# borodark/exmc

Hardware: AMD Instinct MI355X
Metric: leapfrog_steps_per_s (higher is better)
Workload: dtype f64; 1 GPU; eight_schools d=10, 4096 chains/GPU (4096 total), 138450 draws/chain (2769 steps of 50 draws) after one shared 1000-iteration warmup, max_tree_depth 10, target_accept 0.8; draws_per_chain=138450, lanes_per_chain=16, warmup_lanes_per_chain=16, seed=42

## Files before the change

exmc_amd/csrc/exmc_models.hpp:

```cpp
#pragma once

#include "exmc_device.hpp"

namespace exmc {

__device__ __forceinline__ double clamp200(double z) { return fmax(-200.0, fmin(z, 200.0)); }

struct ModelDefaults {
  static constexpr bool kVregMath = false;
  static constexpr bool kCoop = false;
  static constexpr int kExtraLdsDoubles = 0;
  static constexpr int kStageDoubles = 0;
  template <class C>
  __host__ static bool stage_ok(const C&) { return true; }
  static constexpr int kStageRowOffset = 0;
  static constexpr int kLdsDataDoubles = 0;
  static constexpr bool kPipeWarmup = true;
  static constexpr bool kHasPipeWarmup = true;
  static constexpr bool kXRowLds = false;
  static constexpr bool kRowDense = false;
  static constexpr bool kLaneDense = false;
  static constexpr bool kDenseImage = false;
  static constexpr int kDenseLdsDoubles = 0;
  static constexpr int kNutsWavesPerSimd = 1;
  static constexpr bool kRngOrbit = false;
  static constexpr bool kMigrate = false;
  static constexpr double kPrioRateWith = 1.0, kPrioRateWithout = 1.0;
  static constexpr int kPipeNutsLevels = 0;
  static constexpr bool kNutsZigInLds = true;
  static constexpr bool kRegradProposal = false;
  static constexpr int kWgWaves = 0;
  static constexpr int kWgLdsLevels = 1;
  static constexpr int kWgImageDoubles = 0;
  template <class C>
  __host__ __device__ static bool wg_ok(const C&) { return false; }
  static constexpr bool kLeafPairs = false;
  static constexpr bool kLeafPairExp = false;
  static constexpr bool kLeanMomentum = false;
  static constexpr bool kPassExpPairs = false;
  static constexpr bool kOuterLogPair = false;
  static constexpr bool kTreePrefix = false;
};

extern __shared__ double exmc_dyn_lds[];
typedef double exmc_v2d __attribute__((ext_vector_type(2)));
typedef __attribute__((address_space(3))) exmc_v2d lds_v2d;
typedef __attribute__((address_space(3))) double lds_f64_m;
static __device__ const double exmc_logtab_dev[2 * EXMC_LOGTAB_ENTRIES] = {EXMC_LOGTAB_VALUES};
__device__ static __forceinline__ double exmc_log_tab_global(double x) {
  double m;
  int e;
  const int i = exmc_logtab_split(x, &m, &e);
  return exmc_logtab_finish(m, e, exmc_logtab_dev[2 * i], exmc_logtab_dev[2 * i + 1]);
}

struct EightSchoolsConsts {
  double y[8], sg[8], lsg[8];
  double c_mu;
  double c_hc;
  double c1;
};

template <int G>
struct EightSchools : ModelDefaults {
  static constexpr int D = 10;
  static constexpr int DPL = (D + G - 1) / G;
  static constexpr bool kVregMath = (DPL <= 2);
#ifndef EXMC_ES_PIPE_LEVELS
#define EXMC_ES_PIPE_LEVELS 2
#endif
  static constexpr int kPipeNutsLevels = (G == 16) ? EXMC_ES_PIPE_LEVELS : 0;
  static constexpr bool kLeafPairs = (G == 16);
  static constexpr bool kLeafPairExp = (G == 16);
  static constexpr bool kLeanMomentum = (G == 16);
  static constexpr bool kOuterLogPair = (G == 16);
  static constexpr bool kTreePrefix = (G == 16);
  using MM = Math<kVregMath>;
  using Consts = EightSchoolsConsts;
  struct Lane {
    double y[DPL], lsg[DPL];
    Recip sg[DPL];
    Recip five;
    double cc;
  };

  __device__ static __forceinline__ void load(const Consts& c, int l, Lane& ln) {
#pragma unroll
    for (int k = 0; k < DPL; k++) {
      const int i = l + k * G;
      const int j = (i >= 2 && i < D) ? (i - 2) : 0;
      ln.y[k] = c.y[j];
      ln.sg[k] = make_recip(c.sg[j]);
      ln.lsg[k] = c.lsg[j];
    }
    ln.five = make_recip_literal(5.0);
    ln.cc = (l == 0) ? c.c_mu : c.c1;
  }

  __device__ static __forceinline__ double logp_grad(const Consts& c, const Lane& ln, int l,
                                                     const double (&q)[DPL], double (&g)[DPL]) {
    return with_fast_div([&](auto& dv) -> double { return eval(c, ln, l, q, g, dv); });
  }

  template <class DV>
  __device__ static __forceinline__ double eval(const Consts& c, const Lane& ln, int l,
                                                const double (&q)[DPL], double (&g)[DPL], DV& dv) {
    if constexpr (kSeqSum<G, D>) return eval_row(c, ln, l, q, g, dv);
    else return eval_slots(c, ln, l, q, g, dv);
  }

  struct Mid {
    double den, zc, T, lik;
  };
  template <class DV>
  __device__ static __forceinline__ void eval_row_grad(const Consts& c, const Lane& ln, int l,
                                                       const double (&q)[DPL], double (&g)[DPL], DV& dv,
                                                       Mid& m) {
    static_assert(DPL == 1, "one dimension per lane");
    const double mu = group_bcast_c<G, 0>(q[0]);
    const double zraw = group_bcast_c<G, 1>(q[0]);
    const double zc = clamp200(zraw);
    const double tau = MM::exp_pm200(zc);
    const bool isth = (l >= 2) && (l < D);
    const bool l0 = (l == 0), l1 = (l == 1);
    const double th = q[0];
    const double theta = mu + tau * th;
    const double resid = ln.y[0] - theta;
    dv.watch_if(isth, resid);
    dv.watch_if(isth, ln.sg[0].b);
    const double z = dv(resid, ln.sg[0]);
    const double a = dv(z, ln.sg[0]);
    const double Lk = isth ? ((-0.5 * (z * z)) - ln.lsg[0]) : 0.0;
    const double Ak = isth ? a : 0.0;
    const double Bk = isth ? (a * th) : 0.0;
    double lik = 0.0, sa = 0.0, sb = 0.0;
    row_seqsum<D>(lik, sa, sb, Lk, Ak, Bk);
    const double x = l0 ? (mu - 0.0) : tau;
    dv.watch_if(l0, x);
    const double zh = dv(x, ln.five);
    const double zh2 = zh * zh;
    const double w = dv(zh, ln.five);
    const double den = 1.0 + zh2;
    const double dhc = -dv(2.0 * w, den);
    const bool in = (zraw > -200.0) && (zraw < 200.0);
    double g_tau = in ? ((dhc + sb) * tau + 1.0) : 0.0;
    __asm__("" : "+v"(g_tau));
    const double g_mu = (-w) + sa;
    const double g_th = (-th) + a * tau;
    const double u2 = l0 ? zh2 : (th * th);
    g[0] = l0 ? g_mu : (l1 ? g_tau : g_th);
    m.den = den;
    m.zc = zc;
    m.T = -0.5 * (u2 + ln.cc);
    m.lik = lik;
  }
  __device__ static __forceinline__ double eval_row_finish(const Consts& c, int l, const Mid& m, double lg) {
    double t_tau = (c.c_hc - lg) + m.zc;
    __asm__("" : "+v"(t_tau));
    const double T = (l == 1) ? t_tau : m.T;
// ... 1108 lines not shown
          for (int j = 0; j < kAhead - 1; j++) v[j] = *ad[j];
          __builtin_amdgcn_sched_barrier(0);
          exmc_wait_lgkm0();
#pragma unroll
          for (int j = 0; j < kAhead - 1; j++) sj = sj + v[j];
        }
        sj_own[k] = sj;
      }
    } else {
#pragma unroll
      for (int k = 0; k < DPL; k++) {
        double lik = 0.0, f = 0.0, z2s = 0.0, sj = 0.0;
        for (int i = ln.i0[k]; i < ln.i1[k]; i++) sj = sj + obs(alpha_own[k], c.fl[i], c.y[i], lik, f, z2s);
        sj_own[k] = sj;
        if (valid[k]) {
          s[0] = s[0] + lik;
          s[4] = s[4] + f;
          s[5] = s[5] + z2s;
        }
      }
    }
#pragma unroll
    for (int k = 0; k < DPL; k++) {
      const double ar = q[k];
      const double sj = sj_own[k];
      if (valid[k]) {
        s[1] = s[1] + sj;
        s[2] = s[2] + sj * ln.u[k];
        s[3] = s[3] + sj * ar;
      }
      T[k] = -0.5 * (ar * ar + ln.kc[kC1]);
      g[k] = (-ar) + sj * sa;
    }
    if constexpr (G == 64) rs64_allsum6(s);
    else group_allsum_n<G, 6>(s);
    const bool in_a = (zsa_raw > -200.0) && (zsa_raw < 200.0);
    const bool in_y = (zsy_raw > -200.0) && (zsy_raw < 200.0);
    if constexpr (kSpread) {
      constexpr int ks = J / G;
      const int j = l + ks * G;
      const bool is_mu = j == J, is_g = j == J + 1, is_a = j == J + 2, is_y = j == J + 3, is_b = j == J + 4;
      const double v = is_mu ? mu : (is_g ? gam : beta);
      Recip rc;
      rc.b = is_mu ? ln.ten.b : ln.five.b;
      rc.r = is_mu ? ln.ten.r : ln.five.r;
      const double cst = is_mu ? ln.kc[kMu10] : ln.kc[kN5];
      const double sx = is_mu ? s[1] : (is_g ? s[2] : s[4]);
      const double zn = dv(v - 0.0, rc);
      const double Tn = -0.5 * (zn * zn + cst);
      const double gn = (-dv(zn, rc)) + sx;
      const double zc = is_a ? za : zy, zc2 = is_a ? za2 : zy2;
      const double dc = -dv(dv(2.0 * zc, ln.c25), 1.0 + zc2);
      const double ga = in_a ? ((dc + s[3]) * sa + 1.0) : 0.0;
      const double gy = in_y ? ((dc * sy + s[5]) + 1.0) : 0.0;
      const bool is_n = is_mu || is_g || is_b;
      T[ks] = is_n ? Tn : (is_a ? t_sa : (is_y ? t_sy : T[ks]));
      g[ks] = is_n ? gn : (is_a ? ga : (is_y ? gy : g[ks]));
#pragma unroll
      for (int k = 0; k < DPL; k++)
        if (l + k * G >= D) g[k] = 0.0;
      return group_sum_slots<G, DPL>(T, valid, l, s[0]);
    }
    const double zmu = dv(mu - 0.0, ln.ten), zg = dv(gam - 0.0, ln.five), zb = dv(beta - 0.0, ln.five);
#pragma unroll
    for (int k = 0; k < DPL; k++) {
      const int j = l + k * G;
      if (j == J) { T[k] = -0.5 * (zmu * zmu + ln.kc[kMu10]); g[k] = (-dv(zmu, ln.ten)) + s[1]; }
      if (j == J + 1) { T[k] = -0.5 * (zg * zg + ln.kc[kN5]); g[k] = (-dv(zg, ln.five)) + s[2]; }
      if (j == J + 2) { T[k] = t_sa; g[k] = in_a ? ((dsa + s[3]) * sa + 1.0) : 0.0; }
      if (j == J + 3) { T[k] = t_sy; g[k] = in_y ? ((dsy * sy + s[5]) + 1.0) : 0.0; }
      if (j == J + 4) { T[k] = -0.5 * (zb * zb + ln.kc[kN5]); g[k] = (-dv(zb, ln.five)) + s[4]; }
      if (j >= D) g[k] = 0.0;
    }
    return group_sum_slots<G, DPL>(T, valid, l, s[0]);
  }
};

template <class M>
struct RowDenseModel : M {
  static constexpr bool kRowDense = true;
  static constexpr bool kPipeWarmup = false;
  static constexpr bool kOuterLogPair = false;
  static constexpr bool kTreePrefix = false;
  static_assert(M::DPL == 1 && M::D <= 12, "row layout: one dimension per lane, D <= 12");
};

template <class M, int G>
struct LaneDenseModel : M {
  static constexpr bool kLaneDense = true;
  static constexpr bool kPipeWarmup = false;
  static constexpr int kNutsWavesPerSimd = 1;
  static constexpr int kPipeNutsLevels = 0;
  static constexpr bool kDenseImage = M::D * M::D * 8 <= 16 * 1024;
  static constexpr int kDenseLdsDoubles = (64 / G) * 3 * M::D + (kDenseImage ? M::D * M::D + 64 : 0);
  static_assert(G >= 16 && M::DPL * G >= M::D && !M::kCoop, "a lane layout that holds the whole chain");
};

}

#ifdef EXMC_CUSTOM_HEADER
#define EXMC_GEN_HOST static inline
#define EXMC_GEN_FN static __host__ __device__ __forceinline__
static __host__ __device__ __noinline__ double exmc_gen_exp_call(double x) { return exmc_exp(x); }
static __host__ __device__ __noinline__ double exmc_gen_log_call(double x) { return exmc_log(x); }
static __host__ __device__ __noinline__ double exmc_gen_log1p_call(double x) { return exmc_log1p(x); }
static __host__ __device__ __noinline__ double exmc_gen_erf_call(double x) { return exmc_erf(x); }
#define EXMC_GEN_ERF exmc_gen_erf_call
#define EXMC_GENV_ERF exmc_gen_erf_call
#ifdef EXMC_GEN_INLINE_MATH
#define EXMC_GEN_EXP exmc_exp
#define EXMC_GEN_LOG exmc_log
#define EXMC_GEN_LOG1P exmc_log1p
#else
#define EXMC_GEN_EXP exmc_gen_exp_call
#define EXMC_GEN_LOG exmc_gen_log_call
#define EXMC_GEN_LOG1P exmc_gen_log1p_call
#endif
#ifdef EXMC_GENV_CALLED_MATH
#define EXMC_GENV_EXP exmc_gen_exp_call
#define EXMC_GENV_LOG exmc_gen_log_call
#define EXMC_GENV_LOG1P exmc_gen_log1p_call
#else
#define EXMC_GENV_EXP exmc_exp
#define EXMC_GENV_LOG exmc_log
#define EXMC_GENV_LOG1P exmc_log1p
#endif
#ifdef EXMC_GENL_CALLED_MATH
#define EXMC_GENL_EXP exmc_gen_exp_call
#define EXMC_GENL_LOG exmc_gen_log_call
#define EXMC_GENL_LOG1P exmc_gen_log1p_call
#else
#define EXMC_GENL_EXP exmc::Math<true>::exp
#define EXMC_GENL_LOG exmc::Math<true>::log
#define EXMC_GENL_LOG1P exmc_log1p
#endif
#define EXMC_GENL_ERF exmc_gen_erf_call
#define EXMC_GEN_CTX_DECL , int shoff
#define EXMC_GEN_SH(i) exmc::exmc_dyn_lds[shoff + (i)]
#define EXMC_GEN_XROW (EXMC_GEN_LANES == 64 && EXMC_GEN_WAVES_PER_SIMD == 2)
#define EXMC_GEN_ALLSUM(s) exmc::group_allsum_n<EXMC_GEN_LANES, EXMC_GEN_NS, EXMC_GEN_XROW>(s)
#define EXMC_GEN_ALLSUM_W(w) exmc::group_allsum_n<EXMC_GEN_LANES, EXMC_GEN_NW, EXMC_GEN_XROW>(w)
#define EXMC_GEN_BATCH_LOG(n, b) exmc::lane_batch<EXMC_GEN_LANES, n>(b, l, [](double a_) { return EXMC_GENL_LOG(a_); })
#define EXMC_GEN_BATCH_EXP(n, b) exmc::lane_batch<EXMC_GEN_LANES, n>(b, l, [](double a_) { return EXMC_GENL_EXP(a_); })
#define EXMC_GEN_BATCH_LOG1P(n, b) exmc::lane_batch<EXMC_GEN_LANES, n>(b, l, [](double a_) { return EXMC_GENL_LOG1P(a_); })
#define EXMC_GEN_BATCH_RCP(n, b) exmc::lane_batch<EXMC_GEN_LANES, n>(b, l, [](double a_) { return 1.0 / a_; })
#define EXMC_GEN_FENCE() exmc::wave_lds_fence()
#define EXMC_GEN_SCAN_FWD(N, v, m, zo, h, sg, wo)                              \
  do {                                                                        \
    exmc::wave_scan_fwd<N>(v);                                                \
    _Pragma("unroll") for (int k_ = 0; k_ < (N); k_++)                        \
      if (l + 64 * k_ <= (m)) EXMC_GEN_SH((wo) + l + 64 * k_) = (v)[k_];     \
    exmc::wave_lds_fence();                                                   \
  } while (0)
#define EXMC_GEN_SCAN_BWD(N, v, m, zo, sg, we, ww, ga, sz, a0)                 \
  do {                                                                        \
    exmc::wave_scan_bwd<N>(v);                                                \
    double p_[1] = {0.0};                                                     \
    _Pragma("unroll") for (int k_ = 0; k_ < (N); k_++) {                      \
      const int e_ = l + 64 * k_;                                             \
      const bool in_ = e_ >= 1 && e_ <= (m);                                  \
      const double z_ = EXMC_GEN_SH(EXMC_GEN_IT((zo) + e_));                  \
      if (in_) EXMC_GEN_SH((ga) + e_) = (sg) * (v)[k_];                       \
      p_[0] = in_ ? p_[0] + z_ * (v)[k_] : p_[0];                             \
    }                                                                         \
    exmc::group_allsum_n<64, 1, EXMC_GEN_XROW>(p_);                           \
    (sz) = p_[0];                                                             \
// ... 378 lines not shown
```

exmc_amd/csrc/exmc_nuts.hpp:

```cpp
#pragma once

#include <type_traits>

#include "exmc_models.hpp"

#ifndef EXMC_ABLATE
#define EXMC_ABLATE 0
#endif

#ifndef EXMC_PROFILE_SECTIONS
#define EXMC_PROFILE_SECTIONS 0
#endif

namespace exmc {

#ifdef EXMC_XCC_PROBE
__device__ double g_wave_probe[4096 * 5];
#endif

#if EXMC_PROFILE_SECTIONS
__device__ unsigned long long g_prof[16];
#define EXMC_PROF_DECL long long prof_[10] = {0, 0, 0, 0, 0, 0, 0, 0, 0, 0}; long long prof_t_ = clock64();
#define EXMC_PROF(i) { const long long n_ = clock64(); prof_[i] += n_ - prof_t_; prof_t_ = n_; }
#define EXMC_PROF_COUNT(i) { prof_[i] += 1; }
// ... 365 lines not shown
    const uint32_t h1 = (uint32_t)__builtin_amdgcn_ds_bpermute(src, (int)hi[1]);
    const bool up = p >= 64;
    return ((uint64_t)(up ? h1 : h0) << 32) | (uint64_t)(up ? l1 : l0);
  }
  __device__ __forceinline__ Rng state(int p) const {
    auto word = [&](int q) -> uint64_t {
      const int w = q >> 6, i = q & 63;
      const uint32_t l = (w == 0) ? __builtin_amdgcn_readlane((int)lo[0], i) : __builtin_amdgcn_readlane((int)lo[1], i);
      const uint32_t h = (w == 0) ? __builtin_amdgcn_readlane((int)hi[0], i) : __builtin_amdgcn_readlane((int)hi[1], i);
      return ((uint64_t)h << 32) | (uint64_t)l;
    };
    Rng r;
    r.b = word(p);
    r.a = (p == 0) ? a0 : word(p > 0 ? p - 1 : 0);
    return r;
  }
};

#ifndef EXMC_RNG_ORBIT_MARGIN
#define EXMC_RNG_ORBIT_MARGIN 16
#endif

template <class M, int G>
__device__ __forceinline__ void draw_momentum_orbit(const NutsLane<M, G>& L, Rng& rng, double (&z)[M::DPL]) {
  constexpr int D = M::D, DPL = M::DPL;
  constexpr int NORB = D + EXMC_RNG_ORBIT_MARGIN;
#pragma unroll
  for (int k = 0; k < DPL; k++) z[k] = 0.0;
  int pos = 0;
  for (;;) {
    RngOrbit<NORB> orb;
    orb.build(rng);
    const int org = pos;
    int shift = 0;
    bool rebuild = false;
    for (;;) {
      bool fail[DPL];
#pragma unroll
      for (int k = 0; k < DPL; k++) {
        const bool live = L.valid[k] && (L.rank[k] >= pos);
        const int pp = live ? (L.rank[k] - org + shift) : 0;
        double zz;
        const bool acc = normal_fast(rng_scramble(orb.at(pp)), L.zt, zz);
        fail[k] = live && !acc;
        z[k] = (live && acc) ? zz : z[k];
      }
      int j = D;
      if (L.perm == nullptr) {
#pragma unroll
        for (int k = DPL - 1; k >= 0; k--) {
          const unsigned long long m = __ballot(fail[k] ? 1 : 0);
          j = (m != 0) ? (k * G + __ffsll((long long)m) - 1) : j;
        }
      } else {
#pragma unroll
        for (int k = 0; k < DPL; k++) j = fail[k] ? min(j, L.rank[k]) : j;
        j = group_min_i32<G>(j);
      }
      j = __builtin_amdgcn_readfirstlane(j);
      if (j >= D) {
        rng = orb.state(D - org + shift);
        return;
      }
      Rng rj = orb.state(j - org + shift);
      int words = 0;
      const double zz = rng_normal_counted(rj, L.zt, L.nor_r, words);
#pragma unroll
      for (int k = 0; k < DPL; k++) z[k] = (L.rank[k] == j) ? zz : z[k];
      words = __builtin_amdgcn_readfirstlane(words);
      pos = j + 1;
      shift += words - 1;
      if (D - org + shift > NORB - 1) {
        rng = rj;
        rebuild = true;
        break;
      }
    }
    if (!rebuild) return;
    if (pos >= D) return;
  }
}

template <class M, int G>
__device__ __forceinline__ void draw_momentum_lean(const NutsLane<M, G>& L, Rng& rng,
                                                   double (&z)[M::DPL]) {
  constexpr int D = M::D, DPL = M::DPL;
  static_assert(G < 64, "the 64-lane layouts have the orbit form");
  const int base = (threadIdx.x & 63) & ~(G - 1);
#pragma unroll
  for (int k = 0; k < DPL; k++) z[k] = 0.0;
  int pos = 0;
  bool first = true;
  for (;;) {
    Rng r2 = rng;
    uint64_t sb[DPL];
#pragma unroll
    for (int k = 0; k < DPL; k++) sb[k] = 0;
    if (first) {
#pragma nounroll
      for (int i = 0; i < D; i++) {
#pragma unroll
        for (int k = 0; k < DPL; k++) sb[k] = (L.rank[k] == i) ? r2.b : sb[k];
        rng_advance(r2);
      }
    } else {
      const int i0 = wave_min_pos<G>(pos);
#pragma nounroll
      for (int i = i0; i < D; i++) {
        const bool act = i >= pos;
#pragma unroll
        for (int k = 0; k < DPL; k++) sb[k] = (act && (L.rank[k] == i)) ? r2.b : sb[k];
        Rng nx = r2;
        rng_advance(nx);
        r2.a = act ? nx.a : r2.a;
        r2.b = act ? nx.b : r2.b;
      }
    }
    first = false;
    bool fail[DPL];
#pragma unroll
    for (int k = 0; k < DPL; k++) {
      const bool live = L.valid[k] && (L.rank[k] >= pos);
      double zz;
      const bool acc = normal_fast(rng_scramble(sb[k]), L.zt, zz);
      fail[k] = live && !acc;
      z[k] = (live && acc) ? zz : z[k];
    }
    int j = D;
#pragma unroll
    for (int k = DPL - 1; k >= 0; k--) {
      const unsigned long long m = __ballot(fail[k] ? 1 : 0);
      const unsigned long long gm = (m >> base) & ((1ULL << G) - 1ULL);
      j = (gm != 0) ? (k * G + __ffsll((long long)gm) - 1) : j;
    }
    if (__any((j < D) ? 1 : 0) == 0) {
      rng = r2;
      break;
    }
    if (j < D) {
      const int jp = (j > pos) ? j - 1 : j;
      uint64_t bj = 0, bp = 0;
#pragma unroll
      for (int k = 0; k < DPL; k++) {
        bj = (k == j / G) ? sb[k] : bj;
        bp = (k == jp / G) ? sb[k] : bp;
      }
      Rng rj;
      rj.b = __shfl(bj, base | (j & (G - 1)), 64);
      const uint64_t hp = __shfl(bp, base | (jp & (G - 1)), 64);
      rj.a = (j > pos) ? hp : rng.a;
      const double zz = rng_normal(rj, L.zt, L.nor_r);
#pragma unroll
      for (int k = 0; k < DPL; k++) z[k] = (L.rank[k] == j) ? zz : z[k];
      rng = rj;
      pos = j + 1;
    } else {
      rng = r2;
      pos = D;
    }
  }
}

template <class M, int G>
__device__ __forceinline__ void draw_momentum_variates(const NutsLane<M, G>& L, Rng& rng,
                                                       double (&z)[M::DPL]) {
  constexpr int D = M::D, DPL = M::DPL;
  if constexpr (G == 64 && M::kRngOrbit && D + EXMC_RNG_ORBIT_MARGIN <= 128) {
    draw_momentum_orbit<M, G>(L, rng, z);
    return;
  }
  if constexpr (G < 64 && M::kLeanMomentum) {
    if (L.perm == nullptr) {
      draw_momentum_lean<M, G>(L, rng, z);
      return;
    }
  }
  const int base = (threadIdx.x & 63) & ~(G - 1);
#pragma unroll
  for (int k = 0; k < DPL; k++) z[k] = 0.0;
  int pos = 0;
  for (;;) {
    Rng r2 = rng;
    uint64_t sa[DPL], sb[DPL];
#pragma unroll
    for (int k = 0; k < DPL; k++) { sa[k] = 0; sb[k] = 0; }
    const int i0 = wave_min_pos<G>(pos);
#pragma nounroll
    for (int i = i0; i < D; i++) {
      const bool act = (G == 64) || (i >= pos);
#pragma unroll
      for (int k = 0; k < DPL; k++) {
        const bool mine = act && (L.rank[k] == i);
        sa[k] = mine ? r2.a : sa[k];
        sb[k] = mine ? r2.b : sb[k];
      }
      Rng nx = r2;
      rng_advance(nx);
      r2.a = act ? nx.a : r2.a;
      r2.b = act ? nx.b : r2.b;
    }
    bool fail[DPL];
#pragma unroll
    for (int k = 0; k < DPL; k++) {
      const bool live = L.valid[k] && (L.rank[k] >= pos);
      double zz;
      const bool acc = normal_fast(rng_scramble(sb[k]), L.zt, zz);
      fail[k] = live && !acc;
      z[k] = (live && acc) ? zz : z[k];
    }
    int j = D;
    if (L.perm == nullptr) {
#pragma unroll
      for (int k = DPL - 1; k >= 0; k--) {
        const unsigned long long m = __ballot(fail[k] ? 1 : 0);
        const unsigned long long gm = (G == 64) ? m : ((m >> base) & ((1ULL << (G & 63)) - 1ULL));
        j = (gm != 0) ? (k * G + __ffsll((long long)gm) - 1) : j;
      }
    } else {
#pragma unroll
      for (int k = 0; k < DPL; k++) j = fail[k] ? min(j, L.rank[k]) : j;
      j = group_min_i32<G>(j);
    }
    if (__any((j < D) ? 1 : 0) == 0) {
      rng = r2;
      break;
    }
    if (j < D) {
      const int dim = (L.perm == nullptr) ? j : L.perm[j];
      const int ks = dim / G;
      uint64_t aj = 0, bj = 0;
#pragma unroll
      for (int k = 0; k < DPL; k++) {
        aj = (k == ks) ? sa[k] : aj;
        bj = (k == ks) ? sb[k] : bj;
      }
      const int src = base | (dim & (G - 1));
      Rng rj;
      rj.a = __shfl(aj, src, 64);
      rj.b = __shfl(bj, src, 64);
      const double zz = rng_normal(rj, L.zt, L.nor_r);
#pragma unroll
      for (int k = 0; k < DPL; k++) z[k] = (L.rank[k] == j) ? zz : z[k];
// ... 332 lines not shown
#pragma unroll
    for (int k = 0; k < DPL; k++) {
      const double ph = p[k] + h * g[k];
      p[k] = ph;
      q[k] = q[k] + eps_dir * (im[k] * ph);
    }
    f.logp = M::logp_grad(mc, L.ln, L.l, q, g);
#pragma unroll
    for (int k = 0; k < DPL; k++) p[k] = p[k] + h * g[k];
    const double jlp = f.logp - kinetic_energy<G, DPL, M::D, M::kXRowLds>(p, im, L.valid);
    const bool fin = exmc_isfinite(jlp);
    const double dl = jlp - jlp0;
    f.div = fin ? (dl < -1000.0) : true;
    f.lsw = fin ? dl : -1001.0;
    f.acc = f.div ? 0.0 : fmin(1.0, MM::exp_le0(fmin(dl, 0.0)));
#pragma unroll
    for (int k = 0; k < DPL; k++) { f.q[k] = q[k]; f.p[k] = p[k]; f.g[k] = g[k]; }
    pb.put_leaf(which, f);
  };
  auto unit = [&](double eps_dir, bool pair) {
    leap(eps_dir, 0);
    if (pair) leap(eps_dir, 1);
    EXMC_IPROF_COUNT
  };
  bool go_right = rng_uniform(prng) > 0.5;
  EXMC_IPROF(3)
  unit(go_right ? eps : -eps, false);
  EXMC_IPROF(1)
  for (int depth = 0;; depth++) {
    pb.sync();
    EXMC_IPROF(2)
    if (__any(pb.get_alive() ? 1 : 0) == 0) break;
    const double eps_dir = go_right ? eps : -eps;
    const int nunit = (depth == 0) ? 1 : (1 << (depth - 1));
    bool stopped = false;
    for (int i = 1; i < nunit; i++) {
      unit(eps_dir, true);
      EXMC_IPROF(1)
      pb.sync();
      EXMC_IPROF(2)
      if (__any(pb.get_alive() ? 1 : 0) == 0) { stopped = true; break; }
    }
    if (stopped) continue;
#pragma unroll
    for (int k = 0; k < DPL; k++) {
      if (go_right) { qR[k] = q[k]; pR[k] = p[k]; gR[k] = g[k]; }
      else { qL[k] = q[k]; pL[k] = p[k]; gL[k] = g[k]; }
    }
    const int nleaf = 1 << depth;
    for (int i = 0; i < nleaf; i++) rng_advance(prng);
    go_right = rng_uniform(prng) > 0.5;
#pragma unroll
    for (int k = 0; k < DPL; k++) {
      q[k] = go_right ? qR[k] : qL[k];
      p[k] = go_right ? pR[k] : pL[k];
      g[k] = go_right ? gR[k] : gL[k];
    }
    EXMC_IPROF(3)
    unit(go_right ? eps : -eps, true);
    EXMC_IPROF(1)
  }
  {
    double z[DPL];
    const Rng before = next_rng;
    draw_momentum_variates<M, G>(L, next_rng, z);
    pb.put_momentum(z, before, next_rng);
  }
  EXMC_IPROF(3)
  pb.sync();
  EXMC_IPROF(2)
  EXMC_IPROF_FLUSH
  return true;
}

template <int DPL>
struct TreeTop {
  double (&qL)[DPL], (&pL)[DPL], (&gL)[DPL], (&qR)[DPL], (&pR)[DPL], (&gR)[DPL];
  double (&rho)[DPL], (&qp)[DPL], (&gp)[DPL];
  double &logpP, &lsw, &acc;
  int &n, &depth;
  bool &div, &turn, &alive;
};

template <class M, int G>
__device__ __forceinline__ void tree_prefix(const typename M::Consts& mc, const NutsLane<M, G>& L,
                                            double eps, double jlp0, int max_depth, Rng& trng,
                                            TreeTop<M::DPL> T, double (&q)[M::DPL], double (&p)[M::DPL],
                                            double (&g)[M::DPL]) {
  constexpr int DPL = M::DPL;
  using MM = Math<M::kVregMath>;
  static_assert(G >= 11, "one lane per argument of the widest batch");
  static_assert(!M::kRegradProposal, "the proposal's gradient travels with it");
  double u[10];
#pragma unroll
  for (int i = 0; i < 10; i++) u[i] = rng_uniform(trng);
  const bool r0 = u[0] > 0.5, r1 = u[2] > 0.5, r2 = u[5] > 0.5;

  PipeLeaf<DPL> f0, f1, f2, f3, f4, f5, f6;
  auto leap = [&](double eps_dir, PipeLeaf<DPL>& lf) {
    const double h = eps_dir / 2.0;
#pragma unroll
    for (int k = 0; k < DPL; k++) p[k] = p[k] + h * g[k];
    mass_drift<M, G>(L, eps_dir, p, q);
    lf.logp = M::logp_grad(mc, L.ln, L.l, q, g);
#pragma unroll
    for (int k = 0; k < DPL; k++) p[k] = p[k] + h * g[k];
#pragma unroll
    for (int k = 0; k < DPL; k++) { lf.q[k] = q[k]; lf.p[k] = p[k]; lf.g[k] = g[k]; }
  };
  double q1[DPL], g1[DPL], q2[DPL], g2[DPL];
#pragma unroll
  for (int k = 0; k < DPL; k++) { q[k] = T.qL[k]; p[k] = T.pL[k]; g[k] = T.gL[k]; }
  leap(r0 ? eps : -eps, f0);
  const bool same01 = (r0 == r1), same12 = (r1 == r2);
#pragma unroll
  for (int k = 0; k < DPL; k++) {
    q[k] = q1[k] = same01 ? f0.q[k] : T.qL[k];
    p[k] = same01 ? f0.p[k] : T.pL[k];
    g[k] = g1[k] = same01 ? f0.g[k] : T.gL[k];
  }
  leap(r1 ? eps : -eps, f1);
  leap(r1 ? eps : -eps, f2);
#pragma unroll
  for (int k = 0; k < DPL; k++) {
    q[k] = q2[k] = same12 ? f2.q[k] : (same01 ? T.qL[k] : f0.q[k]);
    p[k] = same12 ? f2.p[k] : (same01 ? T.pL[k] : f0.p[k]);
    g[k] = g2[k] = same12 ? f2.g[k] : (same01 ? T.gL[k] : f0.g[k]);
  }
  leap(r2 ? eps : -eps, f3);
  leap(r2 ? eps : -eps, f4);
  leap(r2 ? eps : -eps, f5);
  leap(r2 ? eps : -eps, f6);

  auto scalars = [&](PipeLeaf<DPL>& lf) -> double {
    const double jlp = lf.logp - mass_ke<M, G>(L, lf.p);
    const bool fin = exmc_isfinite(jlp);
    const double dl = jlp - jlp0;
    lf.div = fin ? (dl < -1000.0) : true;
    lf.lsw = fin ? dl : -1001.0;
    return fmin(dl, 0.0);
  };
  double x[11];
  x[0] = scalars(f0); x[1] = scalars(f1); x[2] = scalars(f2); x[3] = scalars(f3);
  x[4] = scalars(f4); x[5] = scalars(f5); x[6] = scalars(f6);
  x[7] = MM::lse_arg(f1.lsw, f2.lsw);
  x[8] = MM::lse_arg(f3.lsw, f4.lsw);
  x[9] = MM::lse_arg(f5.lsw, f6.lsw);
  x[10] = MM::lse_arg(T.lsw, f0.lsw);
  lane_batch<G>(x, L.l, [](double v) { return MM::exp_le0(v); });
  auto accept = [&](PipeLeaf<DPL>& lf, double ex) { lf.acc = lf.div ? 0.0 : fmin(1.0, ex); };
  accept(f0, x[0]); accept(f1, x[1]); accept(f2, x[2]); accept(f3, x[3]);
  accept(f4, x[4]); accept(f5, x[5]); accept(f6, x[6]);

  double y[11] = {1.0 + x[7], 1.0 + x[8], 1.0 + x[9], 1.0 + x[10], u[1], u[3], u[4], u[6], u[7], u[8], u[9]};
  {
    double v[11];
#pragma unroll
    for (int i = 0; i < 11; i++) v[i] = y[i];
    lane_batch<G>(y, L.l, [](double a) { return MM::log_main(a); });
#pragma unroll
    for (int i = 0; i < 4; i++) y[i] = exmc_log_ge1_fix(v[i], y[i]);
#pragma unroll
    for (int i = 4; i < 11; i++) y[i] = exmc_log_unit_fix(v[i], y[i]);
  }
  const double lsw12 = MM::lse_finish(f1.lsw, f2.lsw, y[0]);
  const double lsw34 = MM::lse_finish(f3.lsw, f4.lsw, y[1]);
  const double lsw56 = MM::lse_finish(f5.lsw, f6.lsw, y[2]);
  const double c12 = f1.div ? f1.lsw : lsw12;
  const double c34 = f3.div ? f3.lsw : lsw34;
  const double c56 = f5.div ? f5.lsw : lsw56;

  auto outer = [&](const PipeUnit<DPL>& c, bool go_right, double log1pe, double logu, int depth) {
    if (!T.alive) return;
    const double lsw = MM::lse_finish(T.lsw, c.lsw, log1pe);
    const bool use_sub = logu < (c.lsw - T.lsw);
    if (use_sub) {
      T.logpP = c.logpP;
#pragma unroll
      for (int k = 0; k < DPL; k++) { T.qp[k] = c.qp[k]; T.gp[k] = c.gp[k]; }
    }
    const bool divg = T.div || c.div;
    bool turning = divg || c.turn;
    double rho[DPL];
#pragma unroll
    for (int k = 0; k < DPL; k++) rho[k] = T.rho[k] + c.rho[k];
    if (!turning) {
      double nearp[DPL], farp[DPL], s2[DPL], s3[DPL];
#pragma unroll
      for (int k = 0; k < DPL; k++) {
        nearp[k] = go_right ? T.pR[k] : T.pL[k];
        farp[k] = go_right ? T.pL[k] : T.pR[k];
        s2[k] = T.rho[k] + c.pin[k];
        s3[k] = nearp[k] + c.rho[k];
      }
      bool c1, c23;
      mass_uturn3<M, G>(L, rho, farp, c.p, s2, farp, c.pin, s3, nearp, c.p, c1, c23);
      turning = c1 || c23;
    }
#pragma unroll
    for (int k = 0; k < DPL; k++) {
      T.rho[k] = rho[k];
      if (go_right) { T.qR[k] = c.q[k]; T.pR[k] = c.p[k]; T.gR[k] = c.g[k]; }
      else { T.qL[k] = c.q[k]; T.pL[k] = c.p[k]; T.gL[k] = c.g[k]; }
    }
    T.lsw = lsw;
    T.n += c.n;
    T.acc = T.acc + c.acc;
    T.div = divg;
    T.turn = turning;
    T.depth = depth + 1;
    T.alive = !(T.depth >= max_depth || T.div || T.turn);
  };

  double s0q[DPL], s0g[DPL];
#pragma unroll
  for (int k = 0; k < DPL; k++) { s0q[k] = T.qL[k]; s0g[k] = T.gL[k]; }
  PipeUnit<DPL> c;
  pipe_pair_unit<M, G>(L, f0, f0, false, s0q, s0g, trng, c);
  outer(c, r0, y[3], y[4], 0);

  double w[5] = {f2.lsw - lsw12, f4.lsw - lsw34, f6.lsw - lsw56, MM::lse_arg(lsw34, c56), MM::lse_arg(T.lsw, c12)};
  lane_batch<G>(w, L.l, [](double v) { return MM::exp_le0(v); });
  PipeUnit<DPL> c1, ca, cb;
  pipe_pair_unit<M, G>(L, f1, f2, true, q1, g1, trng, c1, [&](auto, double, double) { return lsw12; },
                       [&](auto, double, double) { return w[0]; }, [&](Rng&) { return u[3]; });
  pipe_pair_unit<M, G>(L, f3, f4, true, q2, g2, trng, ca, [&](auto, double, double) { return lsw34; },
                       [&](auto, double, double) { return w[1]; }, [&](Rng&) { return u[6]; });
  pipe_pair_unit<M, G>(L, f5, f6, true, f4.q, f4.g, trng, cb, [&](auto, double, double) { return lsw56; },
                       [&](auto, double, double) { return w[2]; }, [&](Rng&) { return u[7]; });
  const bool parked = !(ca.div || ca.turn);

  double z[2] = {1.0 + w[3], 1.0 + w[4]};
  {
    const double v0 = z[0], v1 = z[1];
    lane_batch<G>(z, L.l, [](double a) { return MM::log_main(a); });
    z[0] = exmc_log_ge1_fix(v0, z[0]);
    z[1] = exmc_log_ge1_fix(v1, z[1]);
  }
  const double lsw_m = MM::lse_finish(lsw34, c56, z[0]);
  outer(c1, r1, z[1], f1.div ? y[5] : y[6], 1);

  double e[2] = {c56 - lsw_m, MM::lse_arg(T.lsw, parked ? lsw_m : c34)};
  lane_batch<G>(e, L.l, [](double v) { return MM::exp_le0(v); });
  if (parked) {
    const double um = f5.div ? u[7] : u[8];
    const bool use_b = um < e[0];
    if (!use_b) {
      cb.logpP = ca.logpP;
#pragma unroll
      for (int k = 0; k < DPL; k++) { cb.qp[k] = ca.qp[k]; cb.gp[k] = ca.gp[k]; }
    }
    bool turning = cb.div || cb.turn;
    if (!turning) {
      double rho[DPL], s2[DPL], s3[DPL];
#pragma unroll
      for (int k = 0; k < DPL; k++) {
        rho[k] = ca.rho[k] + cb.rho[k];
        s2[k] = ca.rho[k] + cb.pin[k];
        s3[k] = ca.p[k] + cb.rho[k];
      }
      bool t1, t23;
      mass_uturn3<M, G>(L, rho, ca.pin, cb.p, s2, ca.pin, cb.pin, s3, ca.p, cb.p, t1, t23);
      turning = t1 || t23;
#pragma unroll
      for (int k = 0; k < DPL; k++) { cb.rho[k] = rho[k]; cb.pin[k] = ca.pin[k]; }
    }
    cb.lsw = lsw_m;
    cb.acc = ca.acc + cb.acc;
    cb.n = 2 + cb.n;
    cb.turn = turning;
  } else {
    cb = ca;
  }

  const double lu2 = f3.div ? y[7] : (!parked ? y[8] : (f5.div ? y[9] : y[10]));
  outer(cb, r2, MM::log_ge1(1.0 + e[1]), lu2, 2);
}

struct NoIdle {
  __device__ __forceinline__ void operator()() const {}
};

template <class M, int G, int LDSL, class Sink, class Pipe = NoPipe, class Idle = NoIdle>
__device__ __forceinline__ void nuts_run(const typename M::Consts& mc, const NutsLane<M, G>& L,
                                         ChainRegs<M::DPL>& st, int n_draws, double eps,
                                         int max_depth, Sink&& sink, Pipe* pipe = nullptr,
                                         Idle&& idle = Idle{}) {
  constexpr int DPL = M::DPL;
  constexpr int NSLOT = nuts_nslot<M>();
  constexpr bool kRegrad = M::kRegradProposal;
  constexpr int kNodeScalars = NSLOT - 3;
  using MM = Math<M::kVregMath>;
  const int l = L.l;
  const auto& im = L.im;
  double* lstk = L.lstk;
  double* gstk = L.gstk;

  double q[DPL], p[DPL], g[DPL], qold[DPL], gold[DPL];
  double qL[DPL], pL[DPL], gL[DPL], qR[DPL], pR[DPL], gR[DPL];
  double t_rho[DPL], t_qp[DPL], t_gp[DPL];
  double c_rho[DPL], c_pin[DPL], c_qp[DPL], c_gp[DPL];
#pragma unroll
  for (int k = 0; k < DPL; k++) {
    q[k] = p[k] = g[k] = qold[k] = gold[k] = 0.0;
    qL[k] = pL[k] = gL[k] = qR[k] = pR[k] = gR[k] = 0.0;
    t_rho[k] = t_qp[k] = t_gp[k] = c_rho[k] = c_pin[k] = c_qp[k] = c_gp[k] = 0.0;
  }
  double t_logpP = 0.0, t_lsw = 0.0, t_acc = 0.0, jlp0 = 0.0;
  int t_n = 0, t_depth = 0;
  bool t_div = false, t_turn = false, go_right = true;
  double eps_dir = eps;
  Rng trng = st.rng;
  const bool has = L.alive;

  EXMC_PROF_DECL
  for (int draw = 0; draw < n_draws; draw++) {
    EXMC_PROF(8)
    bool alive = has;
    bool have_z = false;
    double z_pre[DPL];
#pragma unroll
    for (int k = 0; k < DPL; k++) z_pre[k] = 0.0;
    if constexpr (Pipe::kOn) {
      if (pipe->pending) {
        pipe->sync();
        pipe->pending = false;
        have_z = pipe->take_momentum(st.rng, z_pre);
      }
    }
    if (has) {
      if (have_z) momentum_from_variates<M, G>(L, z_pre, pL);
      else draw_momentum<M, G>(L, st.rng, pL);
      jlp0 = st.logp - mass_ke<M, G>(L, pL);
      trng = st.rng;
#pragma unroll
      for (int k = 0; k < DPL; k++) {
        qL[k] = qR[k] = t_qp[k] = st.q[k];
        gL[k] = gR[k] = t_gp[k] = st.g[k];
        pR[k] = t_rho[k] = pL[k];
      }
      t_logpP = st.logp;
      t_lsw = 0.0;
      t_acc = 0.0;
      t_n = 0;
      t_div = t_turn = false;
      t_depth = 0;
    }
    if constexpr (Pipe::kOn) {
      pipe->put_start(st.q, pL, st.g, im, eps, jlp0, trng);
      pipe->sync();
    }
    idle();
    EXMC_PROF(0)

    constexpr bool kPrefix = M::kTreePrefix && M::kLeafPairs && Pipe::kTreePrefix && EXMC_ABLATE == 0;
    if constexpr (kPrefix) {
      tree_prefix<M, G>(mc, L, eps, jlp0, max_depth, trng,
                        TreeTop<DPL>{qL, pL, gL, qR, pR, gR, t_rho, t_qp, t_gp, t_logpP, t_lsw, t_acc,
                                     t_n, t_depth, t_div, t_turn, alive},
                        q, p, g);
      EXMC_PROF(7)
    }

    for (int depth = kPrefix ? 3 : 0; Pipe::kOn || __any(alive ? 1 : 0) != 0; depth++) {
      if (alive) {
        const double u = rng_uniform(trng);
        go_right = u > 0.5;
        eps_dir = go_right ? eps : -eps;
#pragma unroll
        for (int k = 0; k < DPL; k++) {
          q[k] = go_right ? qR[k] : qL[k];
          p[k] = go_right ? pR[k] : pL[k];
          g[k] = go_right ? gR[k] : gL[k];
        }
      }
      if constexpr (Pipe::kOn) {
        pipe->put_ctrl(alive, go_right);
        pipe->sync();
        if (__any(alive ? 1 : 0) == 0) break;
      }
      EXMC_PROF(1)

      static_assert(!M::kLeafPairExp || M::kLeafPairs, "kLeafPairExp batches the exponentials of kLeafPairs' pair");
      constexpr bool kOwnPairs = M::kLeafPairs && Pipe::kLeafPairs && EXMC_ABLATE == 0;
      constexpr bool kUnits = Pipe::kOn || kOwnPairs;
      constexpr int kLvl0 = kUnits ? 1 : 0;
      const int nlev = (kUnits && depth > 0) ? depth - 1 : depth;
      const int nleaf = 1 << nlev;
      for (int leaf = 0; leaf < nleaf; leaf++) {
        if constexpr (M::kNutsWavesPerSimd == 2 && !Pipe::kOn) {
          if (L.prio_slot >= 0) {
            const int phase = (int)((clock64() >> 12) & 15);
            const bool mine = (phase < L.prio_duty) == (L.prio_slot == 0);
            if (__builtin_amdgcn_readfirstlane(mine ? 1 : 0)) __builtin_amdgcn_s_setprio(3);
            else __builtin_amdgcn_s_setprio(0);
          }
        }
        if constexpr (Pipe::kOn) {
          if (leaf > 0) pipe->sync();
        }
        if (leaf > 0 && __any(alive ? 1 : 0) == 0) break;
        EXMC_PROF_COUNT(9)
        double logp_new = 0.0, jlp = 0.0;
        PipeLeaf<DPL> la, lb;
        double lsw_ab = 0.0;
        constexpr bool kExpPairs = kOwnPairs && M::kPassExpPairs && G >= 2 && EXMC_ABLATE == 0;
        constexpr bool kLogPair = kOwnPairs && M::kOuterLogPair && G >= 2 && EXMC_ABLATE == 0;
        double e_nx = 0.0, w_b = 0.0;
        auto next_lsw = [&](int nxt) -> double {
          if (nxt >= nlev) return t_lsw;
          if (nxt < LDSL) return ((const lds_f64*)(lstk + ((size_t)nxt * NSLOT + kNodeScalars) * kNutsBlock))[0];
          return gstk[((size_t)(nxt - LDSL) * NSLOT + kNodeScalars) * kNutsBlock];
        };
        (void)next_lsw;
        if constexpr (kOwnPairs) {
          double a_nx = 0.0;
          if constexpr (kExpPairs) a_nx = next_lsw(0);
          leaf_pair<M, G>(mc, L, eps_dir, jlp0, depth > 0, q, p, g, qold, gold, la, lb, lsw_ab, a_nx, w_b, e_nx);
        } else if constexpr (!Pipe::kOn) {
          const double h = eps_dir / 2.0;
#pragma unroll
          for (int k = 0; k < DPL; k++) {
            qold[k] = q[k];
            gold[k] = g[k];
            p[k] = p[k] + h * g[k];
          }
          mass_drift<M, G>(L, eps_dir, p, q);
#if EXMC_ABLATE == 3
          logp_new = 0.0;
#pragma unroll
          for (int k = 0; k < DPL; k++) { g[k] = -q[k]; logp_new = logp_new - 0.5 * q[k] * q[k]; }
          logp_new = group_allsum<G>(logp_new);
#else
          logp_new = M::logp_grad(mc, L.ln, l, q, g);
#endif
#pragma unroll
          for (int k = 0; k < DPL; k++) p[k] = p[k] + h * g[k];
          jlp = logp_new - mass_ke<M, G>(L, p);
        }
// ... 147 lines not shown
          if (!parked) {
#if EXMC_ABLATE == 2
            const double lsw = t_lsw + c_lsw;
            const double u = rng_uniform(trng);
            const bool use_sub = u < 0.5;
#else
            double lsw, u;
            bool use_sub;
            if constexpr (kExpPairs || kLogPair) {
              if (!(kExpPairs && ((below >> nlev) & 1) != 0)) e_nx = MM::exp_le0(MM::lse_arg(t_lsw, c_lsw));
              u = rng_uniform(trng);
              double y[2] = {1.0 + e_nx, u};
              if constexpr (kLogPair) {
                lane_batch<G>(y, l, [](double v) { return MM::log_main(v); });
                y[0] = exmc_log_ge1_fix(1.0 + e_nx, y[0]);
                y[1] = exmc_log_unit_fix(u, y[1]);
              } else {
                y[0] = MM::log_ge1(y[0]);
                y[1] = MM::log_unit(y[1]);
              }
              lsw = MM::lse_finish(t_lsw, c_lsw, y[0]);
              use_sub = y[1] < (c_lsw - t_lsw);
            } else {
              lsw = MM::log_sum_exp(t_lsw, c_lsw);
              u = rng_uniform(trng);
              use_sub = MM::log_unit(u) < (c_lsw - t_lsw);
            }
#endif
            if (use_sub) {
              t_logpP = c_logpP;
#pragma unroll
              for (int k = 0; k < DPL; k++) {
                t_qp[k] = c_qp[k];
                if constexpr (!kRegrad) t_gp[k] = c_gp[k];
              }
            }
            const bool divg = t_div || c_div;
            bool turning = divg || c_turn;
            double rho[DPL];
#pragma unroll
            for (int k = 0; k < DPL; k++) rho[k] = t_rho[k] + c_rho[k];
            if (!turning) {
              double nearp[DPL], farp[DPL], r2[DPL], r3[DPL];
#pragma unroll
              for (int k = 0; k < DPL; k++) {
                nearp[k] = go_right ? pR[k] : pL[k];
                farp[k] = go_right ? pL[k] : pR[k];
                r2[k] = t_rho[k] + c_pin[k];
                r3[k] = nearp[k] + c_rho[k];
              }
              bool c1, c23;
#if EXMC_ABLATE == 1
              c1 = c23 = false;
#else
              mass_uturn3<M, G>(L, rho, farp, p, r2, farp, c_pin, r3, nearp, p, c1, c23);
#endif
              turning = c1 || c23;
            }
#pragma unroll
            for (int k = 0; k < DPL; k++) {
              t_rho[k] = rho[k];
              if (go_right) { qR[k] = q[k]; pR[k] = p[k]; gR[k] = g[k]; }
              else { qL[k] = q[k]; pL[k] = p[k]; gL[k] = g[k]; }
            }
            t_lsw = lsw;
            t_n += c_n;
            t_acc = t_acc + c_acc;
            t_div = divg;
            t_turn = turning;
            t_depth = depth + 1;
            alive = !(t_depth >= max_depth || t_div || t_turn);
          }
          EXMC_PROF(5)
        }
        if constexpr (Pipe::kOn) pipe->put_alive(alive);
      }
    }

    if constexpr (Pipe::kOn) pipe->pending = true;
    if constexpr (kRegrad) {
      (void)M::logp_grad(mc, L.ln, l, t_qp, t_gp);
    }
    if (has) {
      (void)rng_uniform(st.rng);
      st.logp = t_logpP;
#pragma unroll
      for (int k = 0; k < DPL; k++) { st.q[k] = t_qp[k]; st.g[k] = t_gp[k]; }
      sink(draw, st.q, st.logp, t_depth, t_n, t_div, t_acc, jlp0);
    }
    EXMC_PROF(6)
  }
  EXMC_PROF_FLUSH
}

template <class M, int G>
__device__ __forceinline__ void rowdense_load(NutsLane<M, G>& L, const double* cov, const double* chol,
                                              int stride) {
  constexpr int D = M::D;
  const int i = L.l < D ? L.l : 0;
#pragma unroll
  for (int j = 0; j < (M::kRowDense ? D : 1); j++) {
    L.rd.cr[j] = cov ? cov[(size_t)(i * D + j) * stride] : ((i == j) ? 1.0 : 0.0);
    L.rd.ncc[j] = (chol && j > i) ? -chol[(size_t)(j * D + i) * stride] : 0.0;
  }
  L.rd.diag = chol ? chol[(size_t)(i * D + i) * stride] : 1.0;
}

template <class M, int G, int LDSL, bool kZig = true>
__device__ __forceinline__ void lane_setup(NutsLane<M, G>& L, const typename M::Consts& mc,
                                           double* lds, double* stack, const double* inv_mass,
                                           const double* sqrt_inv_mass, const ZigTables& zt,
                                           double nor_r, const FlatOrder& flat = FlatOrder{},
                                           const DenseMass& dm = DenseMass{}) {
  constexpr int D = M::D, DPL = M::DPL;
  const int tid = blockIdx.x * blockDim.x + threadIdx.x;
  L.l = threadIdx.x & (G - 1);
  L.lstk = lds + threadIdx.x;
  L.gstk = stack + (size_t)(tid / kNutsBlock) * nuts_spill_doubles<M, LDSL>() + (tid % kNutsBlock);
  L.zt = zt;
  L.nor_r = nor_r;
  L.alive = true;
  L.prio_slot = -1;
  L.prio_duty = 8;
  M::load(mc, L.l, L.ln);
  if constexpr (M::kExtraLdsDoubles > 0)
    L.ln.sh = lds + (size_t)LDSL * nuts_nslot<M>() * kNutsBlock + nuts_zig_doubles<kZig>();
#pragma unroll
  for (int k = 0; k < DPL; k++) {
    const int i = L.l + k * G;
    L.valid[k] = i < D;
    L.im[k] = (L.valid[k] && inv_mass) ? inv_mass[i] : 1.0;
    L.sim[k] = (L.valid[k] && sqrt_inv_mass) ? sqrt_inv_mass[i] : 1.0;
    L.rank[k] = L.valid[k] ? (flat.rank ? flat.rank[i] : i) : D;
  }
  L.perm = flat.perm;
  L.dm = dm;
  if constexpr (M::kRowDense) rowdense_load<M, G>(L, dm.cov, dm.chol, 1);
  if constexpr (M::kLaneDense) {
    L.ld.covp = dm.covp;
    L.ld.cholp = dm.cholp;
    double* dl = lds + (size_t)LDSL * nuts_nslot<M>() * kNutsBlock + nuts_zig_doubles<kZig>() + M::kExtraLdsDoubles;
    L.ld.xs = dl + (size_t)((threadIdx.x & 63) / G) * 3 * D;
    if constexpr (M::kDenseImage) {
      L.ld.covl = dl + (size_t)(64 / G) * 3 * D;
      if (dm.covp) {
        lane_dense_stage<G, DPL, D>(L.ld, L.l);
        wave_lds_fence();
      }
    }
  }
}

template <class M, int G>
__device__ __forceinline__ void chain_load(const ChainState& s, int C, int chain, int l,
                                           ChainRegs<M::DPL>& st) {
  constexpr int D = M::D, DPL = M::DPL;
  st.logp = s.logp[chain];
  st.rng.a = s.rng[chain];
  st.rng.b = s.rng[(size_t)C + chain];
#pragma unroll
  for (int k = 0; k < DPL; k++) {
    const int i = l + k * G;
    st.q[k] = (i < D) ? s.q[(size_t)i * C + chain] : 0.0;
    st.g[k] = (i < D) ? s.g[(size_t)i * C + chain] : 0.0;
  }
}

// ... 1065 lines not shown
```

Measured before the change: 3.261 billion leapfrog_steps/s.

## Spread RNG stream across a DPP row window for tree prefix and momentum

At the start of the tree prefix, the new code builds a per-row window that holds successive RNG states across the 16 lanes of a DPP row. The ten prefix uniforms and their logs are then computed once per lane and broadcast, instead of every lane advancing the generator serially and taking all the logs itself. The same window is reused to draw the next iteration's momentum in parallel, with a fallback to the serial lean draw when normal rejections move past the window. This cuts serial RNG work and duplicated log evaluations per lane, at the cost of DPP and bpermute traffic, more complex control flow, and reliance on the window covering the draws reached.

```diff
diff --git a/exmc_amd/csrc/exmc_models.hpp b/exmc_amd/csrc/exmc_models.hpp
--- a/exmc_amd/csrc/exmc_models.hpp
+++ b/exmc_amd/csrc/exmc_models.hpp
@@ -40,6 +40,7 @@
   static constexpr bool kPassExpPairs = false;
   static constexpr bool kOuterLogPair = false;
   static constexpr bool kTreePrefix = false;
+  static constexpr bool kRngWindow = false;
 };
 
 extern __shared__ double exmc_dyn_lds[];
@@ -75,6 +76,7 @@
   static constexpr bool kLeanMomentum = (G == 16);
   static constexpr bool kOuterLogPair = (G == 16);
   static constexpr bool kTreePrefix = (G == 16);
+  static constexpr bool kRngWindow = (G == 16);
   using MM = Math<kVregMath>;
   using Consts = EightSchoolsConsts;
   struct Lane {
@@ -1349,6 +1351,7 @@
   static constexpr bool kPipeWarmup = false;
   static constexpr bool kOuterLogPair = false;
   static constexpr bool kTreePrefix = false;
+  static constexpr bool kRngWindow = false;
   static_assert(M::DPL == 1 && M::D <= 12, "row layout: one dimension per lane, D <= 12");
 };
 
diff --git a/exmc_amd/csrc/exmc_nuts.hpp b/exmc_amd/csrc/exmc_nuts.hpp
--- a/exmc_amd/csrc/exmc_nuts.hpp
+++ b/exmc_amd/csrc/exmc_nuts.hpp
@@ -471,15 +471,11 @@
 }
 
 template <class M, int G>
-__device__ __forceinline__ void draw_momentum_lean(const NutsLane<M, G>& L, Rng& rng,
-                                                   double (&z)[M::DPL]) {
+__device__ __forceinline__ void draw_momentum_lean_from(const NutsLane<M, G>& L, Rng& rng,
+                                                        double (&z)[M::DPL], int pos, bool first) {
   constexpr int D = M::D, DPL = M::DPL;
   static_assert(G < 64, "the 64-lane layouts have the orbit form");
   const int base = (threadIdx.x & 63) & ~(G - 1);
-#pragma unroll
-  for (int k = 0; k < DPL; k++) z[k] = 0.0;
-  int pos = 0;
-  bool first = true;
   for (;;) {
     Rng r2 = rng;
     uint64_t sb[DPL];
@@ -547,6 +543,114 @@
       rng = r2;
       pos = D;
     }
+  }
+}
+
+template <class M, int G>
+__device__ __forceinline__ void draw_momentum_lean(const NutsLane<M, G>& L, Rng& rng,
+                                                   double (&z)[M::DPL]) {
+#pragma unroll
+  for (int k = 0; k < M::DPL; k++) z[k] = 0.0;
+  draw_momentum_lean_from<M, G>(L, rng, z, 0, true);
+}
+
+#ifndef EXMC_RNG_WINDOW
+#define EXMC_RNG_WINDOW 14
+#endif
+#ifndef EXMC_RNG_WINDOW_STAGE
+#define EXMC_RNG_WINDOW_STAGE 2
+#endif
+template <int W>
+struct RngRowWindow {
+  static_assert(W >= 11 && W <= 16, "ten uniforms and the state behind them; one DPP row");
+  static constexpr int kOff = 16 - W;
+  uint32_t lo, hi;
+  __device__ __forceinline__ void build(Rng r) {
+    lo = hi = 0;
+#pragma unroll
+    for (int i = 0; i < W; i++) {
+      lo = (uint32_t)__builtin_amdgcn_update_dpp((int)(uint32_t)r.b, (int)lo, 0x101, 0xF, 0xF, false);
+      hi = (uint32_t)__builtin_amdgcn_update_dpp((int)(uint32_t)(r.b >> 32), (int)hi, 0x101, 0xF, 0xF, false);
+      rng_advance(r);
+    }
+  }
+  __device__ __forceinline__ uint64_t own() const { return ((uint64_t)hi << 32) | (uint64_t)lo; }
+  template <int I>
+  __device__ __forceinline__ uint64_t word() const {
+    static_assert(I >= 0 && I < W, "word outside the window");
+    const uint32_t l = (uint32_t)__builtin_amdgcn_mov_dpp((int)lo, 0x150 + kOff + I, 0xF, 0xF, true);
+    const uint32_t h = (uint32_t)__builtin_amdgcn_mov_dpp((int)hi, 0x150 + kOff + I, 0xF, 0xF, true);
+    return ((uint64_t)h << 32) | (uint64_t)l;
+  }
+  template <int I>
+  __device__ __forceinline__ Rng state() const { return Rng{word<I - 1>(), word<I>()}; }
+  __device__ __forceinline__ uint64_t next_rank() const {
+    const uint32_t l = (uint32_t)__builtin_amdgcn_mov_dpp((int)lo, 0x100 + kOff + 1, 0xF, 0xF, true);
+    const uint32_t h = (uint32_t)__builtin_amdgcn_mov_dpp((int)hi, 0x100 + kOff + 1, 0xF, 0xF, true);
+    return ((uint64_t)h << 32) | (uint64_t)l;
+  }
+  __device__ __forceinline__ uint64_t at(int p) const {
+    const int src = (((threadIdx.x & 63) & ~15) | (kOff + p)) << 2;
+    const uint32_t l = (uint32_t)__builtin_amdgcn_ds_bpermute(src, (int)lo);
+    const uint32_t h = (uint32_t)__builtin_amdgcn_ds_bpermute(src, (int)hi);
+    return ((uint64_t)h << 32) | (uint64_t)l;
+  }
+};
+
+template <class M, int G, int W>
+__device__ __forceinline__ void draw_momentum_window(const NutsLane<M, G>& L, const RngRowWindow<W>& win,
+                                                     Rng& rng, double (&z)[M::DPL], int& left) {
+  constexpr int D = M::D;
+  static_assert(G == 16 && M::DPL == 1, "a group is one DPP row with one dimension a lane");
+  static_assert(W >= D + 2, "the state behind the momentum at shift 0");
+  constexpr int kMaxShift = W - D - 2;
+  const int base = (threadIdx.x & 63) & ~(G - 1);
+  const int rank = L.rank[0];
+  z[0] = 0.0;
+  int pos = 0, shift = 0;
+  left = D;
+  uint64_t la = 0, lb = 0;
+  bool flat = true;
+  for (;;) {
+    const bool live = L.valid[0] && (rank >= pos);
+    const uint64_t w = flat ? win.next_rank() : win.at(live ? 1 + rank + shift : 0);
+    double zz;
+    const bool acc = normal_fast(rng_scramble(w), L.zt, zz);
+    const bool fail = live && !acc;
+    z[0] = (live && acc) ? zz : z[0];
+    const unsigned long long m = __ballot(fail ? 1 : 0);
+    const unsigned long long gm = (m >> base) & ((1ULL << G) - 1ULL);
+    const int j = (gm != 0) ? (__ffsll((long long)gm) - 1) : D;
+    if (m == 0) break;
+    flat = false;
+    if (j < D) {
+      const int pj = 1 + j + shift;
+      Rng rj;
+      rj.a = win.at(pj - 1);
+      rj.b = win.at(pj);
+      int words = 0;
+      zz = rng_normal_counted(rj, L.zt, L.nor_r, words);
+      z[0] = (rank == j) ? zz : z[0];
+      shift += words - 1;
+      pos = j + 1;
+      if (shift > kMaxShift) {
+        la = rj.a;
+        lb = rj.b;
+        left = pos;
+        pos = D;
+      }
+    } else {
+      pos = D;
+    }
+  }
+  if (flat) {
+    rng = win.template state<D + 1>();
+  } else {
+    const bool gone = shift > kMaxShift;
+    const int pe = gone ? 1 : D + 1 + shift;
+    const uint64_t ea = win.at(pe - 1), eb = win.at(pe);
+    rng.a = gone ? la : ea;
+    rng.b = gone ? lb : eb;
   }
 }
 
@@ -1045,19 +1149,39 @@
   bool &div, &turn, &alive;
 };
 
-template <class M, int G>
+struct NoRngWindow {
+  static constexpr int kOff = 0;
+};
+template <int I>
+using IntC = std::integral_constant<int, I>;
+
+template <class M, int G, class Win = NoRngWindow>
 __device__ __forceinline__ void tree_prefix(const typename M::Consts& mc, const NutsLane<M, G>& L,
                                             double eps, double jlp0, int max_depth, Rng& trng,
                                             TreeTop<M::DPL> T, double (&q)[M::DPL], double (&p)[M::DPL],
-                                            double (&g)[M::DPL]) {
+                                            double (&g)[M::DPL], Win* win = nullptr) {
   constexpr int DPL = M::DPL;
   using MM = Math<M::kVregMath>;
   static_assert(G >= 11, "one lane per argument of the widest batch");
   static_assert(!M::kRegradProposal, "the proposal's gradient travels with it");
+  constexpr bool kWin = !std::is_same<Win, NoRngWindow>::value;
   double u[10];
-#pragma unroll
-  for (int i = 0; i < 10; i++) u[i] = rng_uniform(trng);
-  const bool r0 = u[0] > 0.5, r1 = u[2] > 0.5, r2 = u[5] > 0.5;
+  double ul = 0.0;
+  if constexpr (kWin) {
+    static_assert(G == 16, "a group is one DPP row");
+    win->build(trng);
+    ul = (double)(rng_scramble(win->own()) >> 5) * 0x1p-53;
+    trng = win->template state<10>();
+  } else {
+#pragma unroll
+    for (int i = 0; i < 10; i++) u[i] = rng_uniform(trng);
+  }
+  auto U = [&](auto ic) -> double {
+    constexpr int I = decltype(ic)::value;
+    if constexpr (kWin) return group_bcast_c<G, Win::kOff + I>(ul);
+    else return u[I];
+  };
+  const bool r0 = U(IntC<0>{}) > 0.5, r1 = U(IntC<2>{}) > 0.5, r2 = U(IntC<5>{}) > 0.5;
 
   PipeLeaf<DPL> f0, f1, f2, f3, f4, f5, f6;
   auto leap = [&](double eps_dir, PipeLeaf<DPL>& lf) {
@@ -1115,8 +1239,31 @@
   accept(f0, x[0]); accept(f1, x[1]); accept(f2, x[2]); accept(f3, x[3]);
   accept(f4, x[4]); accept(f5, x[5]); accept(f6, x[6]);
 
-  double y[11] = {1.0 + x[7], 1.0 + x[8], 1.0 + x[9], 1.0 + x[10], u[1], u[3], u[4], u[6], u[7], u[8], u[9]};
-  {
+  double y[11] = {1.0 + x[7], 1.0 + x[8], 1.0 + x[9], 1.0 + x[10], 0.0, 0.0, 0.0, 0.0, 0.0, 0.0, 0.0};
+  if constexpr (kWin) {
+    constexpr int o = Win::kOff;
+    const int l = L.l;
+    const bool ge1 = (l == o) || (l == o + 2) || (l == o + 5) || (l == o + 10);
+    double a = ul;
+    a = (l == o) ? y[0] : a;
+    a = (l == o + 2) ? y[1] : a;
+    a = (l == o + 5) ? y[2] : a;
+    a = (l == o + 10) ? y[3] : a;
+    const double r = MM::log_main(a);
+    const double v = ge1 ? exmc_log_ge1_fix(a, r) : exmc_log_unit_fix(a, r);
+    y[0] = group_bcast_c<G, o>(v);
+    y[1] = group_bcast_c<G, o + 2>(v);
+    y[2] = group_bcast_c<G, o + 5>(v);
+    y[3] = group_bcast_c<G, o + 10>(v);
+    y[4] = group_bcast_c<G, o + 1>(v);
+    y[5] = group_bcast_c<G, o + 3>(v);
+    y[6] = group_bcast_c<G, o + 4>(v);
+    y[7] = group_bcast_c<G, o + 6>(v);
+    y[8] = group_bcast_c<G, o + 7>(v);
+    y[9] = group_bcast_c<G, o + 8>(v);
+    y[10] = group_bcast_c<G, o + 9>(v);
+  } else {
+    y[4] = u[1]; y[5] = u[3]; y[6] = u[4]; y[7] = u[6]; y[8] = u[7]; y[9] = u[8]; y[10] = u[9];
     double v[11];
 #pragma unroll
     for (int i = 0; i < 11; i++) v[i] = y[i];
@@ -1186,11 +1333,11 @@
   lane_batch<G>(w, L.l, [](double v) { return MM::exp_le0(v); });
   PipeUnit<DPL> c1, ca, cb;
   pipe_pair_unit<M, G>(L, f1, f2, true, q1, g1, trng, c1, [&](auto, double, double) { return lsw12; },
-                       [&](auto, double, double) { return w[0]; }, [&](Rng&) { return u[3]; });
+                       [&](auto, double, double) { return w[0]; }, [&](Rng&) { return U(IntC<3>{}); });
   pipe_pair_unit<M, G>(L, f3, f4, true, q2, g2, trng, ca, [&](auto, double, double) { return lsw34; },
-                       [&](auto, double, double) { return w[1]; }, [&](Rng&) { return u[6]; });
+                       [&](auto, double, double) { return w[1]; }, [&](Rng&) { return U(IntC<6>{}); });
   pipe_pair_unit<M, G>(L, f5, f6, true, f4.q, f4.g, trng, cb, [&](auto, double, double) { return lsw56; },
-                       [&](auto, double, double) { return w[2]; }, [&](Rng&) { return u[7]; });
+                       [&](auto, double, double) { return w[2]; }, [&](Rng&) { return U(IntC<7>{}); });
   const bool parked = !(ca.div || ca.turn);
 
   double z[2] = {1.0 + w[3], 1.0 + w[4]};
@@ -1206,7 +1353,7 @@
   double e[2] = {c56 - lsw_m, MM::lse_arg(T.lsw, parked ? lsw_m : c34)};
   lane_batch<G>(e, L.l, [](double v) { return MM::exp_le0(v); });
   if (parked) {
-    const double um = f5.div ? u[7] : u[8];
+    const double um = f5.div ? U(IntC<7>{}) : U(IntC<8>{});
     const bool use_b = um < e[0];
     if (!use_b) {
       cb.logpP = ca.logpP;
@@ -1275,6 +1422,11 @@
   double eps_dir = eps;
   Rng trng = st.rng;
   const bool has = L.alive;
+  constexpr bool kPrefix = M::kTreePrefix && M::kLeafPairs && Pipe::kTreePrefix && EXMC_ABLATE == 0;
+  constexpr bool kWindow = kPrefix && M::kRngWindow && G == 16 && EXMC_RNG_WINDOW_STAGE >= 1;
+  constexpr bool kWinMomentum = kWindow && EXMC_RNG_WINDOW_STAGE >= 2 && DPL == 1 && M::kLeanMomentum && !M::kRowDense;
+  using Win = RngRowWindow<kWinMomentum ? EXMC_RNG_WINDOW : 11>;
+  Win win{0, 0};
 
   EXMC_PROF_DECL
   for (int draw = 0; draw < n_draws; draw++) {
@@ -1292,8 +1444,19 @@
       }
     }
     if (has) {
-      if (have_z) momentum_from_variates<M, G>(L, z_pre, pL);
-      else draw_momentum<M, G>(L, st.rng, pL);
+      if (have_z) {
+        momentum_from_variates<M, G>(L, z_pre, pL);
+      } else if (kWinMomentum && L.perm == nullptr) {
+        if constexpr (kWinMomentum) {
+          int left = 0;
+          if (draw > 0) draw_momentum_window<M, G>(L, win, st.rng, z_pre, left);
+          if (draw == 0 || __any((left < M::D) ? 1 : 0) != 0)
+            draw_momentum_lean_from<M, G>(L, st.rng, z_pre, left, draw == 0);
+          momentum_from_variates<M, G>(L, z_pre, pL);
+        }
+      } else {
+        draw_momentum<M, G>(L, st.rng, pL);
+      }
       jlp0 = st.logp - mass_ke<M, G>(L, pL);
       trng = st.rng;
 #pragma unroll
@@ -1316,8 +1479,13 @@
     idle();
     EXMC_PROF(0)
 
-    constexpr bool kPrefix = M::kTreePrefix && M::kLeafPairs && Pipe::kTreePrefix && EXMC_ABLATE == 0;
-    if constexpr (kPrefix) {
+    if constexpr (kWindow) {
+      tree_prefix<M, G, Win>(mc, L, eps, jlp0, max_depth, trng,
+                             TreeTop<DPL>{qL, pL, gL, qR, pR, gR, t_rho, t_qp, t_gp, t_logpP, t_lsw, t_acc,
+                                          t_n, t_depth, t_div, t_turn, alive},
+                             q, p, g, &win);
+      EXMC_PROF(7)
+    } else if constexpr (kPrefix) {
       tree_prefix<M, G>(mc, L, eps, jlp0, max_depth, trng,
                         TreeTop<DPL>{qL, pL, gL, qR, pR, gR, t_rho, t_qp, t_gp, t_logpP, t_lsw, t_acc,
                                      t_n, t_depth, t_div, t_turn, alive},
@@ -1631,7 +1799,8 @@
       (void)M::logp_grad(mc, L.ln, l, t_qp, t_gp);
     }
     if (has) {
-      (void)rng_uniform(st.rng);
+      if constexpr (kWindow) st.rng = win.template state<1>();
+      else (void)rng_uniform(st.rng);
       st.logp = t_logpP;
 #pragma unroll
       for (int k = 0; k < DPL; k++) { st.q[k] = t_qp[k]; st.g[k] = t_gp[k]; }
```

New measurement: 3.576 billion leapfrog_steps/s, median of 6. 1.1x the previous value.
